# Nesquiko/Latticeum

Hardware: AMD Instinct MI355X
Metric: fold-steps/sec (Ajtai commit+fold) at d=1024 (higher is better)
Workload: dtype u64 (Goldilocks mod-p integer); 1 GPU; configs[2] at d=1024: commit+fold step, X^1024+1, W=16384, kappa=32, K=15; rho is an input; transcript, linearization, sumchecks, Mz outside the step; d=1024, W=16384, N=81920, kappa=32

## Files before the change

### latticeum_amd/csrc/api_step.hip

```cpp
#include <algorithm>

#include "api_internal.hpp"

namespace {

struct PhaseTimer {
  lf_ctx *c;
  int phase;
  hipEvent_t a = nullptr;
  PhaseTimer(lf_ctx *ctx, int ph) : c(ctx), phase(ph) {
    if (c->timing && hipEventCreate(&a) == hipSuccess) (void)hipEventRecord(a, c->cur);
  }
  ~PhaseTimer() {
    hipEvent_t b = nullptr;
    if (a && hipEventCreate(&b) == hipSuccess) {
      (void)hipEventRecord(b, c->cur);
      c->pending.push_back({a, b, -1 - phase});
    }
  }
};

bool n4k_ok(const Tables *t, int d, int lbs, int K) { return d == 4096 && lbs == 1 && K <= 15 && t->fwd.tw4; }

enum class Decomp { Plain, Fused1024, Fused24, Fused4k };
struct StepPlan {
  Decomp dec = Decomp::Plain;
  FoldPath path = FoldPath::Ntt;
};
StepPlan step_plan(const lf_ajtai *aj, const lf_params *pr, int lbs, const Tables *t, const lf_fold_step_bufs *b) {
  const int d = pr->d, L = pr->L, K = pr->K;
  const bool grouped = aj->Af && aj->geom.Lp == L;
  const bool no_fk = !b->fk[0] && !b->fk[1], no_fck = !b->fk_coeff[0] && !b->fk_coeff[1];
  StepPlan p;
  if (grouped && d == 1024 && lbs == 1 && K <= 15 && t->fwd.mid) {
    p.dec = Decomp::Fused1024;
    p.path = !no_fk ? FoldPath::Coeff1024 : no_fck ? FoldPath::Coeff1024Rows : FoldPath::Rows;
  } else if (grouped && d == 24 && L <= 5) {
    p.dec = Decomp::Fused24;
    p.path = lbs != 1 ? FoldPath::Ntt : no_fk ? FoldPath::Masks24Packed : FoldPath::Masks24;
  } else if (grouped && aj->geom.qperm && n4k_ok(t, d, lbs, K)) {
    p.dec = Decomp::Fused4k;
    p.path = no_fk ? FoldPath::Rows : FoldPath::Ntt;
  }
  return p;
}

uint32_t step_sides(lfk::FusedSides &sd, const uint64_t *const *fc, const lf_fold_step_bufs *b, int extra, int K,
                    bool p0) {
  uint32_t rows = 0;
  sd.nside = 2;
  for (int s = 0; s < 2; s++) {
    sd.f_coeff[s] = fc[s];
    sd.f_coeff_k[s] = b->fk_coeff[s];
    sd.f_k[s] = b->fk[s];
    sd.w_ccs_k[s] = b->wk[s];
    sd.row0[s] = extra + s * (K - 1);
    sd.row_p0[s] = p0 ? extra + 2 * (K - 1) + s : -1;
    for (int k = 1; k < K; k++) rows |= 1u << (sd.row0[s] + k - 1);
    if (p0) rows |= 1u << sd.row_p0[s];
  }
  return rows;
}

int decompose_n4k_sides(lf_ctx *c, const Tables *t, lfk::FusedSides &sd, size_t N, int lb, int L, int K,
                        uint4 *frag = nullptr, int nch = 0) {
  const bool own = !(frag && sd.smg[0]);
  if (c->step.path == FoldPath::Coeff1024 || c->step.path == FoldPath::Coeff1024Rows) c->step = {};
  if (own) LF_TRY(grow(c, c->smg, c->smg_elems, (size_t)sd.nside * N * (frag ? (size_t)K * 256 : 2048)));
  LF_HIP(c, lfk::decompose_n4k(sd, N, lb, L, K, own ? reinterpret_cast<uint64_t *>(c->smg) : nullptr, t->fwd, c->d_err,
                               c->sink, c->ncu, c->cur, frag, nch));
  return LF_OK;
}

int fold_nvec(const lf_params *pr, bool commit_f) { return (commit_f ? 1 : 0) + 2 * (pr->K - 1); }

struct Deferred {
  const uint4 *Ff = nullptr;
  uint64_t *partial = nullptr;
  lfk::OutPtrs dst{};
  lfk::DeadUnits dead{};
  const uint4 *zero80 = nullptr;
  int nvec = 0;
  bool set = false;
};
int grow_dead(lf_ctx *c, size_t need) {
  if (need <= c->dead_elems) return LF_OK;
  LF_TRY(grow(c, c->dead, c->dead_elems, need));
  LF_HIP(c, hipMemsetAsync(c->dead, 0, need, c->cur));
  return LF_OK;
}

int fold_commit(lf_ctx *c, const lf_ajtai *aj, const lf_params *pr, int lb, int lbs, size_t W,
                const lf_fold_step_bufs *b, const uint64_t *wi_f_coeff, const uint64_t *commit_f,
                const lfk::OutPtrs &dst, Deferred *defer = nullptr, const uint32_t *prepacked1 = nullptr) {
  const int d = pr->d, L = pr->L, K = pr->K;
  const size_t N = W * (size_t)L, kappa = aj->kappa;
  const int extra = commit_f ? 1 : 0, nvec = fold_nvec(pr, commit_f != nullptr);
  c->step = {};
  if (2 * K > LF_MAX_VECS || nvec > LF_MAX_VECS) return fail(c, LF_ERR_INVALID_ARG, "2K must be <= 32");
  if (aj->ncols != N) return fail(c, LF_ERR_WRONG_WITNESS_LENGTH, "witness length != Ajtai width");
  Tables *t;
  LF_TRY(get_tables(c, d, t));
  const uint64_t *fc_side[2] = {b->acc_f_coeff, wi_f_coeff};
  const size_t kd = kappa * (size_t)d;
  StepPlan plan = step_plan(aj, pr, lbs, t, b);
  const bool fused = plan.dec == Decomp::Fused1024, fused24 = plan.dec == Decomp::Fused24,
             fused4k = plan.dec == Decomp::Fused4k;
  const bool no_fk = !b->fk[0] && !b->fk[1];
  if (b->planes[0] || b->planes[1]) {
    if (!(fused24 || fused || fused4k) || lbs != 1 || !b->planes[0] || !b->planes[1])
      return fail(c, LF_ERR_INVALID_ARG,
                  "packed planes: d = 24 or the fused d = 1024 / 4096 paths, b_small = 2, both sides");
  }
  const bool packed1024 = plan.path == FoldPath::Coeff1024Rows;
  const bool packed24 = no_fk && fused24;
  StepState st{};
  st.N = N;
  if (packed24) {
    if (lbs != 1) return fail(c, LF_ERR_INVALID_ARG, "packed Phi_72 planes need b_small = 2");
    if (b->fk_coeff[0] || b->fk_coeff[1])
      return fail(c, LF_ERR_INVALID_ARG, "Phi_72: f_k and f_coeff_k are both given or both NULL");
  } else if (no_fk) {
    if (!fused && !fused4k)
      return fail(c, LF_ERR_INVALID_ARG, "f_k buffers may be omitted only on the fused X^1024+1 / X^4096+1 paths");
    if (fused4k && (b->fk_coeff[0] || b->fk_coeff[1]) && !(b->fk_coeff[0] && b->fk_coeff[1]))
      return fail(c, LF_ERR_INVALID_ARG, "f_coeff_k: both sides or neither");
    if (fused && !packed1024 && (!b->fk_coeff[0] || !b->fk_coeff[1]))
      return fail(c, LF_ERR_INVALID_ARG, "f_coeff_k: both sides or neither");
    if (extra + 2 * (K - 1) + 2 > LF_MAX_VECS) return fail(c, LF_ERR_INVALID_ARG, "too many operand rows");
    st.fold_rows.n = 2 * K;
    for (int s2 = 0; s2 < 2; s2++)
      for (int k = 0; k < K; k++) {
        st.fold_rows.row[s2 * K + k] = k > 0 ? extra + s2 * (K - 1) + k - 1 : extra + 2 * (K - 1) + s2;
        st.fold_rows.rho[s2 * K + k] = s2 * K + k;
      }
  } else if (!b->fk[0] || !b->fk[1]) {
    return fail(c, LF_ERR_INVALID_ARG, "f_k: both sides or neither");
  }
  if (plan.dec == Decomp::Plain) {
    if (n4k_ok(t, d, lbs, K)) {
      lfk::FusedSides sd{};
      step_sides(sd, fc_side, b, 0, K, false);
      PhaseTimer pt(c, LF_PHASE_DECOMPOSE);
      LF_TRY(decompose_n4k_sides(c, t, sd, N, lb, L, K));
    } else {
      for (int s = 0; s < 2; s++) {
        PhaseTimer pt(c, LF_PHASE_DECOMPOSE);
        LF_HIP(c, lfk::decompose_witness(fc_side[s], N, d, lb, L, lbs, K, b->fk_coeff[s], b->fk[s], b->wk[s], t->fwd,
                                         c->d_err, c->cur));
      }
    }
    std::vector<const uint64_t *> vecs;
    if (commit_f) vecs.push_back(commit_f);
    for (int s = 0; s < 2; s++)
      for (int k = 1; k < K; k++) vecs.push_back(b->fk[s] + (size_t)k * N * d);
    LF_TRY(grow(c, c->ybuf, c->ybuf_elems, (size_t)nvec * kd));
    LF_TRY(ajtai_launch(c, aj, vecs.data(), nvec, c->ybuf));
    for (int v = 0; v < nvec; v++)
      if (dst.p[v] != c->ybuf + v * kd)
        LF_HIP(c, hipMemcpyAsync(dst.p[v], c->ybuf + v * kd, kd * 8, hipMemcpyDeviceToDevice, c->cur));
    c->step = st;
    return LF_OK;
  }
  LF_TRY(grow(c, c->frag, c->frag_elems, lfk::frag_elems(aj->geom, d)));
  LF_TRY(grow_dead(c, (size_t)aj->geom.nch * 64));
  lfk::FusedSides sd{};
  const uint32_t rows = step_sides(sd, fc_side, b, extra, K, no_fk && !fused24);
  sd.dead = c->dead;
  st.dead_units = {c->dead, rows};
  if (fused4k) {
    for (int s = 0; s < 2 && b->planes[0]; s++) sd.smg[s] = reinterpret_cast<uint32_t *>(b->planes[s]);
    PhaseTimer pt(c, LF_PHASE_DECOMPOSE);
    LF_TRY(decompose_n4k_sides(c, t, sd, N, lb, L, K, c->frag, aj->geom.nch));
  } else if (fused) {
    if (!b->planes[0]) LF_TRY(grow(c, c->smg, c->smg_elems, 2 * N * 512));
    for (int s = 0; s < 2; s++)
      st.smg_side[s] = sd.smg[s] =
          b->planes[0] ? reinterpret_cast<uint32_t *>(b->planes[s]) : c->smg + (size_t)s * N * 512;
    sd.prepacked = prepacked1 && prepacked1 == sd.smg[1] && wi_f_coeff == b->f_coeff ? 2 : 0;
    PhaseTimer pt(c, LF_PHASE_DECOMPOSE);
    LF_HIP(c, lfk::decompose_fused(sd, N, lb, L, K, t->fwd, c->frag, aj->geom.nch, c->d_err,
                                   c->sink, c->ncu, c->cur));
  } else {
    const bool want_masks = lbs == 1;
    if (want_masks && !b->planes[0]) LF_TRY(grow(c, c->fkeys, c->fkeys_elems, 2 * 2 * (size_t)K * N));
    LF_TRY(grow(c, c->smg, c->smg_elems, 2 * N * 12));
    if (lbs != 1) sd.dead = nullptr;
    for (int s = 0; s < 2; s++) {
      sd.smg[s] = c->smg + (size_t)s * N * 12;
      if (want_masks)
        sd.masks[s] = b->planes[s] ? reinterpret_cast<uint2 *>(b->planes[s])
                                   : reinterpret_cast<uint2 *>(c->fkeys) + (size_t)s * K * N;
      st.masks24[s] = sd.masks[s];
    }
    PhaseTimer pt(c, LF_PHASE_DECOMPOSE);
    bool masks = false, dead = false;
    LF_HIP(c, lfk::decompose_phi72_sides(sd, N, lb, L, lbs, K, c->d_err, c->frag, aj->geom.nch, c->cur, &masks,
                                         &dead));
    if (packed24 && !masks) return fail(c, LF_ERR_INVALID_ARG, "packed Phi_72 planes need the wave-local decomposition");
    if (!masks) plan.path = FoldPath::Ntt;
    if (!dead) st.dead_units = lfk::DeadUnits{};
  }
  if (!fused24) st.fold_rows.dead = st.dead_units;
  st.path = plan.path;
  c->step = st;
  lfk::VecPtrs vp{};
  if (commit_f) {
    PhaseTimer pt(c, LF_PHASE_TO_FRAG);
    vp.p[0] = commit_f;
    LF_HIP(c, lfk::to_frag(vp, 1, 0, aj->geom, d, true, c->frag, c->cur));
  }
  LF_TRY(grow(c, c->scratch, c->scratch_elems, partial_elems(aj, nvec)));
  if (defer) {
    defer->Ff = c->frag;
    defer->partial = c->scratch;
    defer->dst = dst;
    defer->dead = c->step.dead_units;
    defer->zero80 = c->zero80;
    defer->nvec = nvec;
    defer->set = true;
    return LF_OK;
  }
  hipEvent_t ea = nullptr, eb = nullptr;
  if (c->timing) {
    LF_HIP(c, hipEventCreate(&ea));
    LF_HIP(c, hipEventCreate(&eb));
  }
  LF_HIP(c, lfk::ajtai_mfma(aj->Af, aj->kr, kappa, aj->geom, d, vp, nvec, true, c->frag, c->scratch, nullptr, c->cur,
                            ea, eb, &dst, &c->step.dead_units, c->zero80));
  if (c->timing) c->pending.push_back({ea, eb, nvec});
  return LF_OK;
}

lfk::OutPtrs fold_dst(const lf_params *pr, const lf_fold_step_bufs *b, size_t kd, uint64_t *commit_cm) {
  lfk::OutPtrs dst{};
  const int extra = commit_cm ? 1 : 0;
  if (commit_cm) dst.p[0] = commit_cm;
  for (int s = 0; s < 2; s++)
    for (int k = 1; k < pr->K; k++) dst.p[extra + s * (pr->K - 1) + k - 1] = b->y[s] + (size_t)k * kd;
  return dst;
}

int fold_finish(lf_ctx *c, const lf_ajtai *aj, const lf_params *pr, int lb, int lbs, size_t W,
                const lf_fold_step_bufs *b, const uint64_t *cm_i) {
  const int d = pr->d, L = pr->L, K = pr->K, nw = 2 * K;
  const size_t N = W * (size_t)L, kappa = aj->kappa;
  Tables *t;
  LF_TRY(get_tables(c, d, t));
  LF_HIP(c, lfk::y0_cm0(b->acc_cm, cm_i, b->y[0], b->y[1], b->rho, kappa, d, lbs, K, b->cm0, c->cur));
  const StepState &st = c->step;
  auto fk_rows = [&] {
    lfk::VecPtrs fx{};
    for (int s = 0; s < 2; s++)
      for (int k = 0; k < K; k++) fx.p[s * K + k] = b->fk[s] + (size_t)k * N * d;
    return fx;
  };
  switch (st.N == N ? st.path : FoldPath::Ntt) {
    case FoldPath::Coeff1024:
    case FoldPath::Coeff1024Rows: {
      const size_t tab_u64 = ((size_t)nw * lfk::FOLD_RT + 7) / 8, aux = (size_t)nw * 1024 + tab_u64 + 1;
      LF_TRY(grow(c, c->fkeys, c->fkeys_elems, 2 * N * (size_t)K * 64 + 2 * N));
      uint32_t *nz = c->fkeys + 2 * N * (size_t)K * 64;
      LF_TRY(grow(c, c->faux, c->faux_elems, aux));
      uint64_t *rc = c->faux;
      uint8_t *tab = reinterpret_cast<uint8_t *>(c->faux + (size_t)nw * 1024);
      int *bad = reinterpret_cast<int *>(c->faux + aux - 1);
      {
        PhaseTimer pt(c, LF_PHASE_FOLD);
        for (int s = 0; s < 2; s++)
          LF_HIP(c, lfk::fold_keys(st.smg_side[s], N, K, c->fkeys + (size_t)s * N * K * 64, c->cur, nz + (size_t)s * N));
        LF_HIP(c, lfk::fold_rho_tables(b->rho, nw, rc, tab, bad, t->inv, c->d_sync, c->cur));
        const int ks_n = lfk::fold_coeff_splits(N, K, c->ncu);
        if (ks_n > 1) LF_TRY(grow(c, c->fpart, c->fpart_elems, (size_t)ks_n * N * 1024));
        const bool in_launch = st.path == FoldPath::Coeff1024Rows;
        const lfk::FoldFallback fb{c->frag, aj->geom.nch, aj->geom.Lp, aj->geom.Wp, st.fold_rows, b->rho, b->f0};
        LF_HIP(c, lfk::fold_coeff(c->fkeys, tab, bad, N, K, b->f0_coeff, c->ncu, c->cur,
                                  ks_n > 1 ? c->fpart : nullptr, in_launch ? &fb : nullptr, L, nz));
        if (!in_launch) LF_HIP(c, lfk::fold(b->rho, fk_rows(), nw, N, d, b->f0, c->cur, bad));
      }
      PhaseTimer pt(c, LF_PHASE_FROM_F);
      LF_HIP(c, lfk::from_fcoeff_n32(b->f0_coeff, W, lb, L, b->f0, b->w_ccs0, t->fwd, bad, c->cur, &t->inv));
      return LF_OK;
    }
    case FoldPath::Masks24:
    case FoldPath::Masks24Packed: {
      const uint2 *m0 = st.masks24[0], *m1 = st.masks24[1];
      LF_TRY(grow(c, c->faux, c->faux_elems, (size_t)nw * 13 + 1));
      uint32_t *rc = reinterpret_cast<uint32_t *>(c->faux);
      int *bad = reinterpret_cast<int *>(c->faux + (size_t)nw * 13);
      {
        PhaseTimer pt(c, LF_PHASE_FOLD);
        LF_HIP(c, lfk::fold_phi72_rho(b->rho, nw, rc, bad, c->cur));
        LF_HIP(c, lfk::fold_phi72_coeff(m0, m1, rc, bad, N, K, L, lb, b->f0_coeff, b->f0, b->w_ccs0, c->cur));
        if (st.path == FoldPath::Masks24Packed)
          LF_HIP(c, lfk::fold_phi72_masks(m0, m1, b->rho, K, N, b->f0, bad, c->cur));
        else
          LF_HIP(c, lfk::fold(b->rho, fk_rows(), nw, N, d, b->f0, c->cur, bad));
      }
      PhaseTimer pt(c, LF_PHASE_FROM_F);
      LF_HIP(c, lfk::from_f(b->f0, N, d, lb, L, b->f0_coeff, b->w_ccs0, t->inv, c->cur, bad));
      return LF_OK;
    }
// ... 125 lines not shown
  b.acc_f_coeff = dafc.p;
  b.rho = drho.p;
  for (int s = 0; s < 2; s++) {
    b.fk_coeff[s] = dfck[s].p;
    b.fk[s] = dfk[s].p;
    b.wk[s] = dwk[s].p;
    b.y[s] = dy.p + (size_t)s * K * kd;
  }
  b.f0 = df0.p;
  b.f0_coeff = df0c.p;
  b.w_ccs0 = dw0.p;
  b.cm0 = dcm0.p;
  LF_TRY(fold_commit(c, aj, pr, lb, lbs, W, &b, dwfc.p, nullptr, fold_dst(pr, &b, kd, nullptr)));
  LF_TRY(fold_finish(c, aj, pr, lb, lbs, W, &b, dcmi.p));
  LF_TRY(download(c, y, dy, 2 * K * kd, repr));
  LF_TRY(download(c, f0, df0, N * d, repr));
  LF_TRY(download(c, f0c, df0c, N * d, repr));
  LF_TRY(download(c, w0, dw0, W * d, repr));
  LF_TRY(download(c, cm0, dcm0, kd, repr));
  return lf_ctx_sync(c);
}

int lf_dev_expand_planes(lf_ctx *c, const lf_params *pr, const uint64_t *planes, size_t N, uint64_t *fck,
                         uint64_t *fk) {
  if (!c) return LF_ERR_INVALID_ARG;
  DevGuard g(c);
  int lb, lbs;
  LF_TRY(check_params(c, pr, lb, lbs));
  const int d = pr->d, K = pr->K;
  if (!planes && N) return fail(c, LF_ERR_INVALID_ARG, "planes is NULL");
  if (lbs != 1) return fail(c, LF_ERR_INVALID_ARG, "packed planes need b_small = 2");
  if (d == 24) {
    LF_HIP(c, lfk::expand_phi72(reinterpret_cast<const uint2 *>(planes), (size_t)K * N, fck, fk, c->cur));
    return LF_OK;
  }
  if ((d != 1024 && d != 4096) || K > 15) return fail(c, LF_ERR_UNSUPPORTED_RING, "packed planes: d = 24, 1024 or 4096");
  if (!fck && !fk) return LF_OK;
  uint64_t *dst = fck ? fck : fk;
  if (d == 1024)
    LF_HIP(c, lfk::expand_sm(reinterpret_cast<const uint32_t *>(planes), N, K, dst, c->cur));
  else
    LF_HIP(c, lfk::expand_sm8(reinterpret_cast<const uint32_t *>(planes), N, K, dst, c->cur));
  if (fk) {
    if (fck) LF_HIP(c, hipMemcpyAsync(fk, fck, (size_t)K * N * d * 8, hipMemcpyDeviceToDevice, c->cur));
    LF_TRY(lf_dev_crt(c, fk, (size_t)K * N, d));
  }
  return LF_OK;
}

int lf_dev_fold_step(lf_ctx *c, const lf_ajtai *aj, const lf_params *pr, size_t W, const lf_fold_step_bufs *b) {
  DevGuard g(c);
  int lb, lbs;
  LF_TRY(step_check(c, aj, pr, W, b, lb, lbs));
  LF_TRY(step_commit(c, aj, pr, W, b, lb, lbs, fold_dst(pr, b, aj->kappa * (size_t)pr->d, b->cm)));
  return fold_finish(c, aj, pr, lb, lbs, W, b, b->cm);
}

int lf_dev_fold_step_batch(lf_ctx *const *cs, int nsteps, const lf_ajtai *aj, const lf_params *pr, size_t W,
                           const lf_fold_step_bufs *const *bs) {
  if (!cs || !bs || !aj || nsteps < 1 || nsteps > LF_MAX_STEPS || !cs[0]) return LF_ERR_INVALID_ARG;
  lf_ctx *c0 = cs[0];
  for (int s = 0; s < nsteps; s++) {
    if (!cs[s] || !bs[s]) return fail(c0, LF_ERR_INVALID_ARG, "null context or step buffers");
    if (cs[s]->device != aj->device) return fail(c0, LF_ERR_INVALID_ARG, "every context must be on the scheme's device");
    for (int t = 0; t < s; t++)
      if (cs[t] == cs[s]) return fail(c0, LF_ERR_INVALID_ARG, "each step needs its own context");
  }
  if (nsteps == 1) return lf_dev_fold_step(c0, aj, pr, W, bs[0]);
  DevGuard g(c0);
  int lb = 0, lbs = 0;
  for (int s = 0; s < nsteps; s++) LF_TRY(step_check(cs[s], aj, pr, W, bs[s], lb, lbs));
  const size_t kd = aj->kappa * (size_t)pr->d;
  Deferred dfr[LF_MAX_STEPS];
  for (int s = 0; s < nsteps; s++) {
    DevGuard gs(cs[s]);
    LF_TRY(step_commit(cs[s], aj, pr, W, bs[s], lb, lbs, fold_dst(pr, bs[s], kd, bs[s]->cm), &dfr[s]));
  }
  const uint4 *ff[LF_MAX_STEPS];
  uint64_t *pp[LF_MAX_STEPS];
  lfk::OutPtrs dd[LF_MAX_STEPS];
  lfk::DeadUnits du[LF_MAX_STEPS];
  int n = 0, nvec = 0;
  for (int s = 0; s < nsteps; s++) {
    if (!dfr[s].set) continue;
    ff[n] = dfr[s].Ff;
    pp[n] = dfr[s].partial;
    dd[n] = dfr[s].dst;
    du[n] = dfr[s].dead;
    nvec = dfr[s].nvec;
    n++;
  }
  for (int s = 0; s < nsteps; s++)
    if (!cs[s]->join) LF_HIP(cs[s], hipEventCreateWithFlags(&cs[s]->join, hipEventDisableTiming));
  if (n) {
    const hipStream_t cst = c0->contract ? c0->contract : c0->cur;
    for (int s = c0->contract ? 0 : 1; s < nsteps; s++) {
      LF_HIP(c0, hipEventRecord(cs[s]->join, cs[s]->cur));
      LF_HIP(c0, hipStreamWaitEvent(cst, cs[s]->join, 0));
    }
    hipEvent_t ea = nullptr, eb = nullptr;
    if (c0->timing) {
      LF_HIP(c0, hipEventCreate(&ea));
      LF_HIP(c0, hipEventCreate(&eb));
    }
    LF_HIP(c0, lfk::ajtai_mfma_steps(aj->Af, aj->kr, aj->kappa, aj->geom, pr->d, nvec, n, ff, pp, dd, cst, ea, eb, du,
                                     c0->zero80));
    if (c0->timing) c0->pending.push_back({ea, eb, nvec, n});
    if (c0->contract) {
      if (!c0->cjoin) LF_HIP(c0, hipEventCreateWithFlags(&c0->cjoin, hipEventDisableTiming));
      LF_HIP(c0, hipEventRecord(c0->cjoin, cst));
      for (int s = 0; s < nsteps; s++) LF_HIP(cs[s], hipStreamWaitEvent(cs[s]->cur, c0->cjoin, 0));
    } else {
      LF_HIP(c0, hipEventRecord(c0->join, c0->cur));
      for (int s = 1; s < nsteps; s++) LF_HIP(cs[s], hipStreamWaitEvent(cs[s]->cur, c0->join, 0));
    }
  }
  for (int s = 0; s < nsteps; s++) {
    DevGuard gs(cs[s]);
    LF_TRY(fold_finish(cs[s], aj, pr, lb, lbs, W, bs[s], bs[s]->cm));
  }
  return LF_OK;
}

size_t lf_fold_step_partial_len(const lf_ajtai *aj, const lf_params *pr) {
  return aj && pr ? (size_t)fold_nvec(pr, true) * aj->kappa * pr->d : 0;
}

int lf_dev_fold_step_partial(lf_ctx *c, const lf_ajtai *aj, const lf_params *pr, size_t W,
                             const lf_fold_step_bufs *b, uint64_t *partial) {
  DevGuard g(c);
  int lb, lbs;
  LF_TRY(step_check(c, aj, pr, W, b, lb, lbs));
  if (!partial) return fail(c, LF_ERR_INVALID_ARG, "null partial buffer");
  const size_t kd = aj->kappa * (size_t)pr->d;
  lfk::OutPtrs dst{};
  for (int v = 0; v < fold_nvec(pr, true); v++) dst.p[v] = partial + v * kd;
  return step_commit(c, aj, pr, W, b, lb, lbs, dst);
}

int lf_dev_fold_step_finish(lf_ctx *c, const lf_ajtai *aj, const lf_params *pr, size_t W,
                            const lf_fold_step_bufs *b, const uint64_t *partial_sum) {
  DevGuard g(c);
  int lb, lbs;
  LF_TRY(step_check(c, aj, pr, W, b, lb, lbs));
  if (!partial_sum) return fail(c, LF_ERR_INVALID_ARG, "null partial sum");
  const size_t kd = aj->kappa * (size_t)pr->d;
  const lfk::OutPtrs dst = fold_dst(pr, b, kd, b->cm);
  for (int v = 0; v < fold_nvec(pr, true); v++)
    LF_HIP(c, hipMemcpyAsync(dst.p[v], partial_sum + v * kd, kd * 8, hipMemcpyDeviceToDevice, c->cur));
  return fold_finish(c, aj, pr, lb, lbs, W, b, b->cm);
}

int lf_dev_decompose_commit(lf_ctx *c, const lf_ajtai *aj, const lf_params *pr, size_t W,
                            const lf_fold_step_bufs *b) {
  DevGuard g(c);
  int lb, lbs;
  LF_TRY(step_check(c, aj, pr, W, b, lb, lbs));
  if (!b->acc_f_coeff || !b->f_coeff || !b->acc_cm || !b->cm || !b->y[0] || !b->y[1] || !b->wk[0] || !b->wk[1])
    return fail(c, LF_ERR_INVALID_ARG, "decompose_commit: missing buffer");
  const size_t kd = aj->kappa * (size_t)pr->d;
  LF_TRY(fold_commit(c, aj, pr, lb, lbs, W, b, b->f_coeff, nullptr, fold_dst(pr, b, kd, nullptr)));
  for (int s = 0; s < 2; s++)
    LF_HIP(c, lfk::commit_y0(s ? b->cm : b->acc_cm, b->y[s], aj->kappa, pr->d, lbs, pr->K, c->cur));
  return LF_OK;
}

int lf_dev_fold_combine(lf_ctx *c, const lf_ajtai *aj, const lf_params *pr, size_t W, const lf_fold_step_bufs *b) {
  DevGuard g(c);
  int lb, lbs;
  LF_TRY(step_check(c, aj, pr, W, b, lb, lbs));
  if (!b->rho || !b->f0 || !b->f0_coeff || !b->w_ccs0 || !b->cm0) return fail(c, LF_ERR_INVALID_ARG, "fold_combine: missing buffer");
  return fold_finish(c, aj, pr, lb, lbs, W, b, b->cm);
}

int lf_dev_fold_step_sharded(lf_ctx *c, const lf_ajtai *aj, const lf_params *pr, size_t W,
                             const lf_fold_step_bufs *b, lf_comm *cm) {
  DevGuard g(c);
  int lb, lbs;
  LF_TRY(step_check(c, aj, pr, W, b, lb, lbs));
  if (!cm || !cm->comm) return lf_dev_fold_step(c, aj, pr, W, b);
  const size_t len = lf_fold_step_partial_len(aj, pr);
  LF_TRY(grow(c, c->stage, c->stage_elems, len));
  LF_TRY(lf_dev_fold_step_partial(c, aj, pr, W, b, c->stage));
  LF_TRY(allreduce_modp(c, cm, c->stage, len));
  return lf_dev_fold_step_finish(c, aj, pr, W, b, c->stage);
}

}
```

### latticeum_amd/csrc/kernels.hip

```cpp
#include <cstdlib>
#include <cstring>

#include "digits.hpp"
#include "frag.hpp"
#include "kernels.hpp"
#include "ring.hpp"

namespace lfk {

using gl::Acc;

template <bool FWD>
__global__ void __launch_bounds__(256) k_phi72_transform(uint64_t *data, size_t n) {
  size_t e = blockIdx.x * (size_t)blockDim.x + threadIdx.x;
  if (e >= n) return;
  uint64_t c[24];
  const ulonglong2 *src = reinterpret_cast<const ulonglong2 *>(data + e * 24);
#pragma unroll
  for (int i = 0; i < 12; i++) {
    ulonglong2 v = src[i];
    c[2 * i] = v.x;
    c[2 * i + 1] = v.y;
  }
  if (FWD)
// ... 683 lines not shown
      uint64_t c[3];
      c[0] = gl::add(gl::cacc_reduce(q.s00), gl::mul_pow2(gl::cacc_reduce(q.s0n), 40));
      c[1] = gl::add(gl::cacc_reduce(q.s1), gl::mul_pow2(gl::cacc_reduce(q.s1n), 40));
      c[2] = gl::cacc_reduce(q.s2);
#pragma unroll
      for (int off = 8; off < 64; off <<= 1)
#pragma unroll
        for (int k = 0; k < 3; k++) c[k] = gl::add(c[k], __shfl_xor(c[k], off));
      if (ph == 0 && i0 + r < (int)kappa && v0 + v < nvec) {
        uint64_t *o = partial + (((size_t)js * nvec + v0 + v) * kappa + i0 + r) * 24 + 3 * slot;
        o[0] = c[0];
        o[1] = c[1];
        o[2] = c[2];
      }
    }
}

__global__ void k_sum_planes(const uint64_t *partial, int nsplit, size_t len, uint64_t *out,
                             size_t out_stride_vec, size_t per_vec) {
  size_t i = blockIdx.x * (size_t)blockDim.x + threadIdx.x;
  if (i >= len) return;
  Acc a;
  gl::acc_zero(a);
  for (int s = 0; s < nsplit; s++) gl::acc_add(a, partial[(size_t)s * len + i]);
  size_t v = i / per_vec, r = i % per_vec;
  out[v * out_stride_vec + r] = gl::acc_reduce(a);
}

__global__ void __launch_bounds__(256) k_sum_planes_to(const uint64_t *partial, int nsplit, size_t len, int nvec,
                                                      OutPtrs out) {
  __shared__ uint64_t part[3][64];
  const int o = threadIdx.x & 63, g = threadIdx.x >> 6;
  const size_t i = blockIdx.x * (size_t)64 + o;
  const bool ok = i < len * nvec;
  Acc a;
  gl::acc_zero(a);
  if (ok)
    for (int s = g; s < nsplit; s += 4) gl::acc_add(a, partial[(size_t)s * len * nvec + i]);
  const uint64_t v = gl::acc_reduce(a);
  if (g > 0) part[g - 1][o] = v;
  __syncthreads();
  if (g == 0 && ok) out.p[i / len][i % len] = gl::add(gl::add(v, part[0][o]), gl::add(part[1][o], part[2][o]));
}

__global__ void k_commit_y0(const uint64_t *cm, uint64_t *y, size_t n, int lbs, int K) {
  size_t c = blockIdx.x * (size_t)blockDim.x + threadIdx.x;
  if (c >= n) return;
  uint64_t acc = 0;
  for (int k = K - 1; k >= 1; k--) acc = gl::mul_pow2(gl::add(acc, y[(size_t)k * n + c]), lbs);
  y[c] = gl::sub(cm[c], acc);
}

constexpr int Y0_KMAX = 16;
__global__ void k_y0_cm0(const uint64_t *cm0s, const uint64_t *cm1s, uint64_t *y0, uint64_t *y1,
                         const uint64_t *rho, size_t n, int d, int lbs, int K, uint64_t *cm0) {
  const size_t c = blockIdx.x * (size_t)blockDim.x + threadIdx.x;
  if (c >= n) return;
  const int s = c % d;
  gl::CAcc a;
  gl::cacc_zero(a);
#pragma unroll
  for (int side = 0; side < 2; side++) {
    uint64_t *y = side ? y1 : y0;
    const uint64_t *rs = rho + (size_t)side * K * d + s;
    uint64_t yv[Y0_KMAX], rv[Y0_KMAX];
#pragma unroll
    for (int k = 1; k < Y0_KMAX; k++)
      if (k < K) {
        yv[k] = y[(size_t)k * n + c];
        rv[k] = rs[(size_t)k * d];
      }
    uint64_t acc = 0;
#pragma unroll
    for (int k = Y0_KMAX - 1; k >= 1; k--)
      if (k < K) {
        gl::cacc_mad(a, rv[k], yv[k]);
        acc = gl::mul_pow2(gl::add(acc, yv[k]), lbs);
      }
    const uint64_t v0 = gl::sub((side ? cm1s : cm0s)[c], acc);
    y[c] = v0;
    gl::cacc_mad(a, rs[0], v0);
  }
  cm0[c] = gl::cacc_reduce(a);
}

__global__ void __launch_bounds__(256) k_y0_cm0_phi72(const uint64_t *cm0s, const uint64_t *cm1s, uint64_t *y0,
                                                     uint64_t *y1, const uint64_t *rho, size_t nslots, int lbs,
                                                     int K, uint64_t *cm0) {
  __shared__ uint64_t part[16][16][9];
  const int q = threadIdx.x & 15, ul = threadIdx.x >> 4;
  const size_t u = blockIdx.x * (size_t)16 + ul;
  const bool ok = u < nslots;
  const size_t n = nslots * 3;
  const int s = u % 8;
  ring::Fq3Acc a;
  ring::fq3acc_zero(a);
  uint64_t hs[2][3] = {{0, 0, 0}, {0, 0, 0}};
  if (ok)
    for (int side = 0; side < 2; side++) {
      const uint64_t *y = side ? y1 : y0;
      for (int k = q > 0 ? q : 16; k < K; k += 16) {
        const uint64_t *v = y + (size_t)k * n + 3 * u, *r = rho + ((size_t)side * K + k) * 24 + 3 * s;
        ring::fq3acc_mad(a, r[0], r[1], r[2], v[0], v[1], v[2]);
        const int e = (int)(((long long)k * lbs) % 192);
#pragma unroll
        for (int c = 0; c < 3; c++) hs[side][c] = gl::add(hs[side][c], gl::mul_pow2(v[c], e));
      }
    }
  uint64_t cc[3];
  ring::fq3acc_final(a, cc);
#pragma unroll
  for (int c = 0; c < 3; c++) {
    part[ul][q][c] = cc[c];
    part[ul][q][3 + c] = hs[0][c];
    part[ul][q][6 + c] = hs[1][c];
  }
  __syncthreads();
  if (q != 0 || !ok) return;
  uint64_t t[9];
#pragma unroll
  for (int c = 0; c < 9; c++) t[c] = part[ul][0][c];
  for (int l = 1; l < 16; l++)
#pragma unroll
    for (int c = 0; c < 9; c++) t[c] = gl::add(t[c], part[ul][l][c]);
  ring::Fq3Acc a0;
  ring::fq3acc_zero(a0);
  for (int side = 0; side < 2; side++) {
    uint64_t *y = side ? y1 : y0;
    const uint64_t *cm = (side ? cm1s : cm0s) + 3 * u, *r = rho + (size_t)side * K * 24 + 3 * s;
    uint64_t v0[3];
#pragma unroll
    for (int c = 0; c < 3; c++) {
      v0[c] = gl::sub(cm[c], t[3 + 3 * side + c]);
// ... 608 lines not shown
}
size_t ajtai_partial_elems(size_t kappa, size_t ncols, int d, int nvec) {
  size_t nsplit = ajtai_nsplit(ncols, d, nvec);
  return nsplit * (size_t)nvec * kappa * (size_t)d;
}

hipError_t ajtai_commit(const uint64_t *A, size_t kappa, size_t ncols, int d, const VecPtrs &fv,
                        int nvec, uint64_t *partial, uint64_t *cm, hipStream_t st, hipEvent_t ev0,
                        hipEvent_t ev1) {
  if (nvec <= 0 || nvec > LF_MAX_VECS) return hipErrorInvalidValue;
  const int nsplit = ajtai_nsplit(ncols, d, nvec);
  const size_t jchunk = (ncols + nsplit - 1) / nsplit;
  if (ev0) (void)hipEventRecord(ev0, st);
  if (d == 24) {
    constexpr int R = 2, V = 2;
    const int nvt = (nvec + V - 1) / V;
    dim3 grid(nsplit / 4, (unsigned)((kappa + R - 1) / R), nvt);
    hipLaunchKernelGGL((k_ajtai_phi72<R, V>), grid, dim3(256), 0, st, A, kappa, ncols, fv, nvec, jchunk,
                       partial);
  } else if (nvec == 1) {
    constexpr int R = 8, V = 1;
    AjtaiGrid g{(d + 255) / 256, (int)((kappa + R - 1) / R), nsplit, 1};
    hipLaunchKernelGGL((k_ajtai_nega<R, V>), dim3(g.blocks()), dim3(256), 0, st, A, kappa, ncols, d, fv,
                       nvec, jchunk, g, partial);
  } else {
    constexpr int R = 4, V = 4;
    AjtaiGrid g{(d + 255) / 256, (int)((kappa + R - 1) / R), nsplit, (nvec + V - 1) / V};
    hipLaunchKernelGGL((k_ajtai_nega<R, V>), dim3(g.blocks()), dim3(256), 0, st, A, kappa, ncols, d, fv,
                       nvec, jchunk, g, partial);
  }
  hipError_t e = hipGetLastError();
  if (e != hipSuccess) return e;
  if (ev1) (void)hipEventRecord(ev1, st);
  const size_t len = (size_t)nvec * kappa * d;
  hipLaunchKernelGGL(k_sum_planes, dim3(blocks(len, 256)), dim3(256), 0, st, partial, nsplit, len, cm,
                     kappa * (size_t)d, kappa * (size_t)d);
  return hipGetLastError();
}

hipError_t sum_planes(const uint64_t *partial, int nsplit, size_t len, uint64_t *out, hipStream_t st) {
  if (len == 0) return hipSuccess;
  hipLaunchKernelGGL(k_sum_planes, dim3(blocks(len, 256)), dim3(256), 0, st, partial, nsplit, len, out, len, len);
  return hipGetLastError();
}

hipError_t sum_planes_to(const uint64_t *partial, int nsplit, size_t len, int nvec, const OutPtrs &out,
                         hipStream_t st) {
  if (len == 0 || nvec < 1) return hipSuccess;
  hipLaunchKernelGGL(k_sum_planes_to, dim3(blocks(len * nvec, 64)), dim3(256), 0, st, partial, nsplit, len, nvec,
                     out);
  return hipGetLastError();
}

hipError_t y0_cm0(const uint64_t *cm0s, const uint64_t *cm1s, uint64_t *y0, uint64_t *y1, const uint64_t *rho,
                  size_t kappa, int d, int lbs, int K, uint64_t *cm0, hipStream_t st) {
  const size_t n = kappa * (size_t)d;
  if (n == 0) return hipSuccess;
  if (K < 1 || K > Y0_KMAX) return hipErrorInvalidValue;
  if (d == 24) {
    hipLaunchKernelGGL(k_y0_cm0_phi72, dim3(blocks(kappa * 8, 16)), dim3(256), 0, st, cm0s, cm1s, y0, y1, rho,
                       kappa * 8, lbs, K, cm0);
    return hipGetLastError();
  }
  hipLaunchKernelGGL(k_y0_cm0, dim3(blocks(n, 256)), dim3(256), 0, st, cm0s, cm1s, y0, y1, rho, n, d, lbs, K, cm0);
  return hipGetLastError();
}

hipError_t commit_y0(const uint64_t *cm, uint64_t *y, size_t kappa, int d, int lbs, int K,
                     hipStream_t st) {
  size_t n = kappa * (size_t)d;
  if (n == 0) return hipSuccess;
  hipLaunchKernelGGL(k_commit_y0, dim3(blocks(n, 256)), dim3(256), 0, st, cm, y, n, lbs, K);
  return hipGetLastError();
}

hipError_t fold(const uint64_t *rho, const VecPtrs &x, int nwit, size_t n, int d, uint64_t *out,
                hipStream_t st, const int *run_if) {
  if (n == 0) return hipSuccess;
  if (nwit <= 0 || nwit > LF_MAX_VECS) return hipErrorInvalidValue;
  if (d == 24) {
    unsigned nb = blocks(n * 8, 256);
    if (run_if && nb > 1024) nb = 1024;
    hipLaunchKernelGGL(k_fold_phi72, dim3(nb), dim3(256), 0, st, rho, x, nwit, n, out, run_if);
  } else {
    unsigned nb = blocks(n * d / 2, 256);
    if (run_if && nb > 8192) nb = 8192;
    hipLaunchKernelGGL(k_fold_nega, dim3(nb), dim3(256), 0, st, rho, x, nwit, n, d, out, run_if);
  }
  return hipGetLastError();
}

hipError_t p2_permute(uint64_t *states, size_t n, hipStream_t st, int rounds) {
  if (n == 0) return hipSuccess;
  if (rounds < 0 || rounds > 30) return hipErrorInvalidValue;
  hipLaunchKernelGGL(k_p2_permute, dim3(blocks(n, 256)), dim3(256), 0, st, states, n, rounds);
  return hipGetLastError();
}

hipError_t fill_uniform(uint64_t *out, size_t n, uint64_t seed, hipStream_t st) {
  if (n == 0) return hipSuccess;
  hipLaunchKernelGGL(k_fill_uniform, dim3(grid_cap(blocks(n, 256))), dim3(256), 0, st, out, n, seed);
  return hipGetLastError();
}

hipError_t modp_sum(const uint64_t *in, int nparts, size_t len, uint64_t *out, hipStream_t st) {
  if (len == 0) return hipSuccess;
  hipLaunchKernelGGL(k_modp_sum, dim3(blocks(len, 256)), dim3(256), 0, st, in, nparts, len, out);
  return hipGetLastError();
}

hipError_t rot_lin(const uint64_t *rho_coeff, const uint64_t *theta, int n, int d, uint64_t *v0, hipStream_t st) {
  if (n < 1 || (d != 24 && (d < 2 || (d & (d - 1))))) return hipErrorInvalidValue;
  const int comp = d == 24 ? 3 : 1;
  hipLaunchKernelGGL(k_rot_lin, dim3((unsigned)(d * comp)), dim3(256), 0, st, rho_coeff, theta, n, d, comp, v0);
  return hipGetLastError();
}

// ... 13 lines not shown
```

### latticeum_amd/csrc/kernels.hpp

```cpp
#pragma once
#include <hip/hip_runtime.h>
#include <stddef.h>
#include <stdint.h>

#include "ring.hpp"

#define LF_MAX_VECS 32
#define LF_MAX_KTILES 4
#define LF_MAX_STEPS 8

namespace lfk {

struct VecPtrs {
  const uint64_t *p[LF_MAX_VECS];
};
struct OutPtrs {
  uint64_t *p[LF_MAX_VECS];
};

struct DeadUnits {
  const uint8_t *flags = nullptr;
  uint32_t rows = 0;
};
struct StepOps {
  const uint4 *Ff[LF_MAX_STEPS];
  uint64_t *partial[LF_MAX_STEPS];
  OutPtrs dst[LF_MAX_STEPS];
  DeadUnits dead[LF_MAX_STEPS];
  const uint4 *zero80 = nullptr;
};

hipError_t transform(uint64_t *data, size_t n, int d, bool fwd, const ring::NegaTables &tb,
                     hipStream_t st);
hipError_t slot_mul(const uint64_t *a, const uint64_t *b, uint64_t *out, size_t n, int d,
                    hipStream_t st);
hipError_t mont(uint64_t *x, size_t n, bool to, hipStream_t st);
hipError_t from_w_ccs(const uint64_t *w_ccs, size_t W, int d, int lb, int L, uint64_t *f_coeff,
                      uint64_t *f, const ring::NegaTables &fwd, const ring::NegaTables &inv, int *err,
                      hipStream_t st, uint32_t *smg = nullptr);
hipError_t from_f(const uint64_t *f, size_t N, int d, int lb, int L, uint64_t *f_coeff,
                  uint64_t *w_ccs, const ring::NegaTables &inv, hipStream_t st, const int *run_if = nullptr);
hipError_t decompose_witness(const uint64_t *f_coeff, size_t N, int d, int lb, int L, int lbs, int K,
                             uint64_t *f_coeff_k, uint64_t *f_k, uint64_t *w_ccs_k,
                             const ring::NegaTables &fwd, int *err, hipStream_t st, uint4 *frag = nullptr,
                             int nch = 0, int row0 = 0);
int ajtai_nsplit(size_t ncols, int d, int nvec);
size_t ajtai_partial_elems(size_t kappa, size_t ncols, int d, int nvec);
hipError_t ajtai_commit(const uint64_t *A, size_t kappa, size_t ncols, int d, const VecPtrs &fv,
                        int nvec, uint64_t *partial, uint64_t *cm, hipStream_t st,
                        hipEvent_t ev0 = nullptr, hipEvent_t ev1 = nullptr);
hipError_t commit_y0(const uint64_t *cm, uint64_t *y, size_t kappa, int d, int lbs, int K,
                     hipStream_t st);
hipError_t fold(const uint64_t *rho, const VecPtrs &x, int nwit, size_t n, int d, uint64_t *out,
                hipStream_t st, const int *run_if = nullptr);
hipError_t p2_permute(uint64_t *states, size_t n, hipStream_t st, int rounds = 30);
hipError_t fill_uniform(uint64_t *out, size_t n, uint64_t seed, hipStream_t st);
hipError_t modp_sum(const uint64_t *in, int nparts, size_t len, uint64_t *out, hipStream_t st);

hipError_t rot_lin(const uint64_t *rho_coeff, const uint64_t *theta, int n, int d, uint64_t *v0, hipStream_t st);
hipError_t limb_split(const uint64_t *x, size_t n, uint64_t *lo, uint64_t *hi, hipStream_t st);
hipError_t limb_join(const uint64_t *lo, const uint64_t *hi, size_t n, uint64_t *out, hipStream_t st);

hipError_t sum_planes(const uint64_t *partial, int nsplit, size_t len, uint64_t *out, hipStream_t st);
hipError_t sum_planes_to(const uint64_t *partial, int nsplit, size_t len, int nvec, const OutPtrs &out,
                         hipStream_t st);
hipError_t y0_cm0(const uint64_t *cm0s, const uint64_t *cm1s, uint64_t *y0, uint64_t *y1, const uint64_t *rho,
                  size_t kappa, int d, int lbs, int K, uint64_t *cm0, hipStream_t st);

struct FragGeom {
  int Lp;
  size_t Wp;
  int nch;
  int qperm = 0;
};
FragGeom frag_geom(size_t ncols, int Lp);
int mfma_dim(int d);
size_t frag_elems(const FragGeom &g, int d);
int mfma_ktiles(size_t kappa);
int mfma_nsplit(const FragGeom &g, int d);
size_t mfma_scratch_elems(const FragGeom &g, int d, size_t kappa, int nvec);
hipError_t to_frag(const VecPtrs &rows, int nrows, int row0, const FragGeom &g, int d, bool vmajor, uint4 *frag,
                   hipStream_t st);
hipError_t ajtai_rowsums(const uint64_t *A, size_t kappa, size_t ncols, int d, uint64_t *kr, uint64_t *tmp,
                         hipStream_t st);
size_t ajtai_rowsums_elems(size_t kappa, int d);
hipError_t ajtai_mfma(const uint4 *Af, const uint64_t *kr, size_t kappa, const FragGeom &g, int d, const VecPtrs &fv,
                      int nvec,
                      bool f_ready, uint4 *Ff, uint64_t *partial, uint64_t *cm, hipStream_t st,
                      hipEvent_t ev0 = nullptr, hipEvent_t ev1 = nullptr, const OutPtrs *dst = nullptr,
                      const DeadUnits *dead = nullptr, const uint4 *zero80 = nullptr);
hipError_t ajtai_mfma_steps(const uint4 *Af, const uint64_t *kr, size_t kappa, const FragGeom &g, int d, int nvec,
                            int nsteps,
                            const uint4 *const *Ff, uint64_t *const *partial, const OutPtrs *dst, hipStream_t st,
                            hipEvent_t ev0 = nullptr, hipEvent_t ev1 = nullptr, const DeadUnits *dead = nullptr,
                            const uint4 *zero80 = nullptr);

size_t witness_split_w();
hipError_t transform_n32(uint64_t *data, size_t n, bool fwd, const ring::NegaTables &tb, hipStream_t st,
                         const uint64_t *src = nullptr);
hipError_t from_w_ccs_n32(const uint64_t *w_ccs, size_t W, int lb, int L, uint64_t *f_coeff, uint64_t *f,
                          const ring::NegaTables &fwd, const ring::NegaTables &inv, int *err, hipStream_t st,
                          uint32_t *smg = nullptr);
hipError_t from_f_n32(const uint64_t *f, size_t W, int lb, int L, uint64_t *f_coeff, uint64_t *w_ccs,
                      const ring::NegaTables &inv, hipStream_t st, const int *run_if = nullptr);
hipError_t decompose_n32(const uint64_t *f_coeff, size_t N, int lb, int L, int K, uint64_t *f_coeff_k,
                         uint64_t *f_k, uint64_t *w_ccs_k, const ring::NegaTables &fwd, int *err,
                         hipStream_t st);
struct FusedSides {
  const uint64_t *f_coeff[2];
  uint64_t *f_coeff_k[2], *f_k[2], *w_ccs_k[2];
  int row0[2];
  int nside;
  int row_p0[2] = {-1, -1};
  uint2 *masks[2] = {nullptr, nullptr};
  uint32_t *smg[2] = {nullptr, nullptr};
  uint8_t *dead = nullptr;
  int prepacked = 0;
};
struct FoldRows {
  int row[LF_MAX_VECS];
// ... 142 lines not shown
```

Measured before the change: 58.59 fold-steps/s.

## Derive commitment from digit-0 plane instead of separately committing f

On the fused d=1024/4096 paths, the separate to_frag and commit of the full witness f is skipped. The digit-0 plane's commitment row is written into y[1] and cm1 is reconstructed as y0 plus the weighted sum of higher-digit commitments inside the y0_cm0 kernel. This removes one operand row from the Ajtai MFMA commit and its fragment conversion, relying on commitment linearity. It adds a templated kernel variant and changes which row feeds the fold.

Result: faster. 59.48 fold-steps/s, median of 6 (+1.5%).

```diff
diff --git a/latticeum_amd/csrc/api_step.hip b/latticeum_amd/csrc/api_step.hip
--- a/latticeum_amd/csrc/api_step.hip
+++ b/latticeum_amd/csrc/api_step.hip
@@ -45,8 +45,19 @@
   return p;
 }
 
+bool z_plane0(const lf_ajtai *aj, const lf_params *pr, int lbs, const Tables *t, const lf_fold_step_bufs *b) {
+  const Decomp dec = step_plan(aj, pr, lbs, t, b).dec;
+  return dec == Decomp::Fused1024 || dec == Decomp::Fused4k;
+}
+int z_plane0(lf_ctx *c, const lf_ajtai *aj, const lf_params *pr, int lbs, const lf_fold_step_bufs *b, bool &z0) {
+  Tables *t;
+  LF_TRY(get_tables(c, pr->d, t));
+  z0 = z_plane0(aj, pr, lbs, t, b);
+  return LF_OK;
+}
+
 uint32_t step_sides(lfk::FusedSides &sd, const uint64_t *const *fc, const lf_fold_step_bufs *b, int extra, int K,
-                    bool p0) {
+                    bool p0, bool z0 = false) {
   uint32_t rows = 0;
   sd.nside = 2;
   for (int s = 0; s < 2; s++) {
@@ -55,9 +66,9 @@
     sd.f_k[s] = b->fk[s];
     sd.w_ccs_k[s] = b->wk[s];
     sd.row0[s] = extra + s * (K - 1);
-    sd.row_p0[s] = p0 ? extra + 2 * (K - 1) + s : -1;
+    sd.row_p0[s] = z0 && s == 1 ? 0 : p0 ? extra + 2 * (K - 1) + s : -1;
     for (int k = 1; k < K; k++) rows |= 1u << (sd.row0[s] + k - 1);
-    if (p0) rows |= 1u << sd.row_p0[s];
+    if (sd.row_p0[s] >= 0) rows |= 1u << sd.row_p0[s];
   }
   return rows;
 }
@@ -107,6 +118,7 @@
   const bool fused = plan.dec == Decomp::Fused1024, fused24 = plan.dec == Decomp::Fused24,
              fused4k = plan.dec == Decomp::Fused4k;
   const bool no_fk = !b->fk[0] && !b->fk[1];
+  const bool z0 = commit_f && z_plane0(aj, pr, lbs, t, b);
   if (b->planes[0] || b->planes[1]) {
     if (!(fused24 || fused || fused4k) || lbs != 1 || !b->planes[0] || !b->planes[1])
       return fail(c, LF_ERR_INVALID_ARG,
@@ -131,7 +143,8 @@
     st.fold_rows.n = 2 * K;
     for (int s2 = 0; s2 < 2; s2++)
       for (int k = 0; k < K; k++) {
-        st.fold_rows.row[s2 * K + k] = k > 0 ? extra + s2 * (K - 1) + k - 1 : extra + 2 * (K - 1) + s2;
+        const int row_p0 = z0 && s2 == 1 ? 0 : extra + 2 * (K - 1) + s2;
+        st.fold_rows.row[s2 * K + k] = k > 0 ? extra + s2 * (K - 1) + k - 1 : row_p0;
         st.fold_rows.rho[s2 * K + k] = s2 * K + k;
       }
   } else if (!b->fk[0] || !b->fk[1]) {
@@ -165,7 +178,7 @@
   LF_TRY(grow(c, c->frag, c->frag_elems, lfk::frag_elems(aj->geom, d)));
   LF_TRY(grow_dead(c, (size_t)aj->geom.nch * 64));
   lfk::FusedSides sd{};
-  const uint32_t rows = step_sides(sd, fc_side, b, extra, K, no_fk && !fused24);
+  const uint32_t rows = step_sides(sd, fc_side, b, extra, K, no_fk && !fused24, z0);
   sd.dead = c->dead;
   st.dead_units = {c->dead, rows};
   if (fused4k) {
@@ -205,7 +218,7 @@
   st.path = plan.path;
   c->step = st;
   lfk::VecPtrs vp{};
-  if (commit_f) {
+  if (commit_f && !z0) {
     PhaseTimer pt(c, LF_PHASE_TO_FRAG);
     vp.p[0] = commit_f;
     LF_HIP(c, lfk::to_frag(vp, 1, 0, aj->geom, d, true, c->frag, c->cur));
@@ -232,22 +245,23 @@
   return LF_OK;
 }
 
-lfk::OutPtrs fold_dst(const lf_params *pr, const lf_fold_step_bufs *b, size_t kd, uint64_t *commit_cm) {
+lfk::OutPtrs fold_dst(const lf_params *pr, const lf_fold_step_bufs *b, size_t kd, uint64_t *commit_cm,
+                      bool z0 = false) {
   lfk::OutPtrs dst{};
   const int extra = commit_cm ? 1 : 0;
-  if (commit_cm) dst.p[0] = commit_cm;
+  if (commit_cm) dst.p[0] = z0 ? b->y[1] : commit_cm;
   for (int s = 0; s < 2; s++)
     for (int k = 1; k < pr->K; k++) dst.p[extra + s * (pr->K - 1) + k - 1] = b->y[s] + (size_t)k * kd;
   return dst;
 }
 
 int fold_finish(lf_ctx *c, const lf_ajtai *aj, const lf_params *pr, int lb, int lbs, size_t W,
-                const lf_fold_step_bufs *b, const uint64_t *cm_i) {
+                const lf_fold_step_bufs *b, uint64_t *cm_i, bool cm1_out = false) {
   const int d = pr->d, L = pr->L, K = pr->K, nw = 2 * K;
   const size_t N = W * (size_t)L, kappa = aj->kappa;
   Tables *t;
   LF_TRY(get_tables(c, d, t));
-  LF_HIP(c, lfk::y0_cm0(b->acc_cm, cm_i, b->y[0], b->y[1], b->rho, kappa, d, lbs, K, b->cm0, c->cur));
+  LF_HIP(c, lfk::y0_cm0(b->acc_cm, cm_i, b->y[0], b->y[1], b->rho, kappa, d, lbs, K, b->cm0, c->cur, cm1_out));
   const StepState &st = c->step;
   auto fk_rows = [&] {
     lfk::VecPtrs fx{};
@@ -479,8 +493,10 @@
   DevGuard g(c);
   int lb, lbs;
   LF_TRY(step_check(c, aj, pr, W, b, lb, lbs));
-  LF_TRY(step_commit(c, aj, pr, W, b, lb, lbs, fold_dst(pr, b, aj->kappa * (size_t)pr->d, b->cm)));
-  return fold_finish(c, aj, pr, lb, lbs, W, b, b->cm);
+  bool z0;
+  LF_TRY(z_plane0(c, aj, pr, lbs, b, z0));
+  LF_TRY(step_commit(c, aj, pr, W, b, lb, lbs, fold_dst(pr, b, aj->kappa * (size_t)pr->d, b->cm, z0)));
+  return fold_finish(c, aj, pr, lb, lbs, W, b, b->cm, z0);
 }
 
 int lf_dev_fold_step_batch(lf_ctx *const *cs, int nsteps, const lf_ajtai *aj, const lf_params *pr, size_t W,
@@ -499,9 +515,11 @@
   for (int s = 0; s < nsteps; s++) LF_TRY(step_check(cs[s], aj, pr, W, bs[s], lb, lbs));
   const size_t kd = aj->kappa * (size_t)pr->d;
   Deferred dfr[LF_MAX_STEPS];
+  bool z0[LF_MAX_STEPS];
   for (int s = 0; s < nsteps; s++) {
     DevGuard gs(cs[s]);
-    LF_TRY(step_commit(cs[s], aj, pr, W, bs[s], lb, lbs, fold_dst(pr, bs[s], kd, bs[s]->cm), &dfr[s]));
+    LF_TRY(z_plane0(cs[s], aj, pr, lbs, bs[s], z0[s]));
+    LF_TRY(step_commit(cs[s], aj, pr, W, bs[s], lb, lbs, fold_dst(pr, bs[s], kd, bs[s]->cm, z0[s]), &dfr[s]));
   }
   const uint4 *ff[LF_MAX_STEPS];
   uint64_t *pp[LF_MAX_STEPS];
@@ -544,7 +562,7 @@
   }
   for (int s = 0; s < nsteps; s++) {
     DevGuard gs(cs[s]);
-    LF_TRY(fold_finish(cs[s], aj, pr, lb, lbs, W, bs[s], bs[s]->cm));
+    LF_TRY(fold_finish(cs[s], aj, pr, lb, lbs, W, bs[s], bs[s]->cm, z0[s]));
   }
   return LF_OK;
 }
@@ -572,10 +590,12 @@
   LF_TRY(step_check(c, aj, pr, W, b, lb, lbs));
   if (!partial_sum) return fail(c, LF_ERR_INVALID_ARG, "null partial sum");
   const size_t kd = aj->kappa * (size_t)pr->d;
-  const lfk::OutPtrs dst = fold_dst(pr, b, kd, b->cm);
+  bool z0;
+  LF_TRY(z_plane0(c, aj, pr, lbs, b, z0));
+  const lfk::OutPtrs dst = fold_dst(pr, b, kd, b->cm, z0);
   for (int v = 0; v < fold_nvec(pr, true); v++)
     LF_HIP(c, hipMemcpyAsync(dst.p[v], partial_sum + v * kd, kd * 8, hipMemcpyDeviceToDevice, c->cur));
-  return fold_finish(c, aj, pr, lb, lbs, W, b, b->cm);
+  return fold_finish(c, aj, pr, lb, lbs, W, b, b->cm, z0);
 }
 
 int lf_dev_decompose_commit(lf_ctx *c, const lf_ajtai *aj, const lf_params *pr, size_t W,
diff --git a/latticeum_amd/csrc/kernels.hip b/latticeum_amd/csrc/kernels.hip
--- a/latticeum_amd/csrc/kernels.hip
+++ b/latticeum_amd/csrc/kernels.hip
@@ -759,7 +759,8 @@
 }
 
 constexpr int Y0_KMAX = 16;
-__global__ void k_y0_cm0(const uint64_t *cm0s, const uint64_t *cm1s, uint64_t *y0, uint64_t *y1,
+template <bool CM1>
+__global__ void k_y0_cm0(const uint64_t *cm0s, uint64_t *cm1s, uint64_t *y0, uint64_t *y1,
                          const uint64_t *rho, size_t n, int d, int lbs, int K, uint64_t *cm0) {
   const size_t c = blockIdx.x * (size_t)blockDim.x + threadIdx.x;
   if (c >= n) return;
@@ -784,8 +785,14 @@
         gl::cacc_mad(a, rv[k], yv[k]);
         acc = gl::mul_pow2(gl::add(acc, yv[k]), lbs);
       }
-    const uint64_t v0 = gl::sub((side ? cm1s : cm0s)[c], acc);
-    y[c] = v0;
+    uint64_t v0;
+    if (CM1 && side) {
+      v0 = y[c];
+      cm1s[c] = gl::add(v0, acc);
+    } else {
+      v0 = gl::sub((side ? cm1s : cm0s)[c], acc);
+      y[c] = v0;
+    }
     gl::cacc_mad(a, rs[0], v0);
   }
   cm0[c] = gl::cacc_reduce(a);
@@ -1500,17 +1507,23 @@
   return hipGetLastError();
 }
 
-hipError_t y0_cm0(const uint64_t *cm0s, const uint64_t *cm1s, uint64_t *y0, uint64_t *y1, const uint64_t *rho,
-                  size_t kappa, int d, int lbs, int K, uint64_t *cm0, hipStream_t st) {
+hipError_t y0_cm0(const uint64_t *cm0s, uint64_t *cm1s, uint64_t *y0, uint64_t *y1, const uint64_t *rho,
+                  size_t kappa, int d, int lbs, int K, uint64_t *cm0, hipStream_t st, bool cm1_out) {
   const size_t n = kappa * (size_t)d;
   if (n == 0) return hipSuccess;
-  if (K < 1 || K > Y0_KMAX) return hipErrorInvalidValue;
+  if (K < 1 || K > Y0_KMAX || (cm1_out && d == 24)) return hipErrorInvalidValue;
+  if (cm1_out) {
+    hipLaunchKernelGGL(k_y0_cm0<true>, dim3(blocks(n, 256)), dim3(256), 0, st, cm0s, cm1s, y0, y1, rho, n, d, lbs, K,
+                       cm0);
+    return hipGetLastError();
+  }
   if (d == 24) {
     hipLaunchKernelGGL(k_y0_cm0_phi72, dim3(blocks(kappa * 8, 16)), dim3(256), 0, st, cm0s, cm1s, y0, y1, rho,
                        kappa * 8, lbs, K, cm0);
     return hipGetLastError();
   }
-  hipLaunchKernelGGL(k_y0_cm0, dim3(blocks(n, 256)), dim3(256), 0, st, cm0s, cm1s, y0, y1, rho, n, d, lbs, K, cm0);
+  hipLaunchKernelGGL(k_y0_cm0<false>, dim3(blocks(n, 256)), dim3(256), 0, st, cm0s, cm1s, y0, y1, rho, n, d, lbs, K,
+                     cm0);
   return hipGetLastError();
 }
 
diff --git a/latticeum_amd/csrc/kernels.hpp b/latticeum_amd/csrc/kernels.hpp
--- a/latticeum_amd/csrc/kernels.hpp
+++ b/latticeum_amd/csrc/kernels.hpp
@@ -64,8 +64,8 @@
 hipError_t sum_planes(const uint64_t *partial, int nsplit, size_t len, uint64_t *out, hipStream_t st);
 hipError_t sum_planes_to(const uint64_t *partial, int nsplit, size_t len, int nvec, const OutPtrs &out,
                          hipStream_t st);
-hipError_t y0_cm0(const uint64_t *cm0s, const uint64_t *cm1s, uint64_t *y0, uint64_t *y1, const uint64_t *rho,
-                  size_t kappa, int d, int lbs, int K, uint64_t *cm0, hipStream_t st);
+hipError_t y0_cm0(const uint64_t *cm0s, uint64_t *cm1s, uint64_t *y0, uint64_t *y1, const uint64_t *rho,
+                  size_t kappa, int d, int lbs, int K, uint64_t *cm0, hipStream_t st, bool cm1_out = false);
 
 struct FragGeom {
   int Lp;
```
